# niveathika/siddhi

Measured on AMD Instinct MI355X. Metric: events/sec ingested + matches/sec (partitioned pattern, 1–8 GPU); % HBM peak, higher is better.
Workload: dtype f64; 1 GPU; P3; events_per_gpu=100000000, keys_per_gpu=10000000, micro_batch=50000896, call_size=1024, parallelism=key-sharded x1, input=prepartitioned

## Files before the change

### siddhi_amd/csrc/engine_pattern.hip

```cpp
#include <algorithm>
#include <unordered_map>
#include <cmath>
#include <cstdio>
#include <cstdlib>

#include "engine.h"
#include "knobs.h"
#include "pattern_common.h"

namespace shd {

using namespace pat;

namespace {

template <bool FAST>
__global__ __launch_bounds__(kBlock) void k_prepare(const PrepArgs* __restrict__ ap, int64_t n_ext, int64_t stride,
                                                    uint32_t* __restrict__ k32, uint64_t* __restrict__ k64,
                                                    uint32_t* __restrict__ pv, int32_t* __restrict__ tso,
                                                    PrepAgg* __restrict__ blk) {
  const PrepArgs& a = *ap;
  const DExprSet es = a.es;
  PrepAcc acc;
  const int64_t tbase = a.x.batch.ts[0];
// ... 160 lines not shown
      int64_t q = p + 1;
      int32_t j = -1;
      uint32_t fm = 0;
      int64_t ra = -1, rb = -1;
      const uint8_t st = walk_partial<true, false, HASH ? 4 : 1>(a, es, n_ext, ld, pv_row(pvp), k, tsi, q, pq, tq,
                                                                 kq, tsi, false, j, steps, viol, fm, ra, rb);
      if (st == ST_DEFER) {
        out = PS_DEFER;
        match_row[p] = (int32_t)q;
        nd++;
      } else if (st == ST_OPEN) {
        out = PS_OPEN;
        no++;
        if (a.logical == 2) match_row[p] = and_open_code(a, pv_row(pvp));
      } else if (st == ST_PRUNED) {
        pruned++;
      }
    }
    pst[p] = out;
  };
  const GlobalPos<K64, TS64> ld{skey32, skey64, spv, sts32, sts64, tbase, a.partitioned};
  for (int64_t p = t0 + threadIdx.x; p < t1; p += kBlock) visit(p, ld);
  scan_block_reduce(steps, pruned, viol, nm, no, blk, blockIdx.x, bcnt, blockIdx.x, gridDim.x, false, nd);
}

__global__ __launch_bounds__(kBlock) void k_gather_bpos(const ExtRows* __restrict__ xp, const uint32_t* spv,
                                                       int64_t n_ext) {
  const ExtRows& x = *xp;
  for (int64_t p = (int64_t)blockIdx.x * kBlock + threadIdx.x; p < n_ext; p += (int64_t)gridDim.x * kBlock) {
    const int64_t r = pv_row(spv[p]);
    const uint32_t m = r < x.C ? x.apos_mask : (x.bpos_mask | x.apos_mask);
    for (int c = 0; c < x.batch.ncols; c++) {
      if (!((m >> c) & 1u)) continue;
      const Val v = r < x.C ? col_load(x.carry, r, c) : col_load(x.batch, r - x.C, c);
      switch (x.bpos.type[c]) {
        case SHD_T_STRING: case SHD_T_INT: case SHD_T_FLOAT: ((uint32_t*)x.bpos.col[c])[p] = (uint32_t)v.b; break;
        case SHD_T_LONG: case SHD_T_DOUBLE: ((uint64_t*)x.bpos.col[c])[p] = v.b; break;
        case SHD_T_BOOL: ((uint8_t*)x.bpos.col[c])[p] = (uint8_t)v.b; break;
      }
      ((uint8_t*)x.bpos.nul[c])[p] = (uint8_t)v.null;
    }
  }
}

__global__ __launch_bounds__(kBlock) void k_block_sum(const ScanArgs* __restrict__ ap, int64_t n_ext,
                                                     const uint32_t* __restrict__ skey32,
// ... 410 lines not shown
  } else if constexpr (MODE == 1) {
    for (int64_t p = t0 + threadIdx.x; p < t1; p += kBlock)
      if (pst[p] == PS_DEFER) resume_one(p);
  } else {
    for (int64_t c0 = t0; c0 < t1; c0 += kBlock * 16) {
      const int64_t pb = c0 + (int64_t)threadIdx.x * 16;
      if (pb >= t1) continue;
      const uint4 raw = *reinterpret_cast<const uint4*>(pst + pb);
      const uint32_t wv[4] = {raw.x, raw.y, raw.z, raw.w};
      uint32_t hit = 0;
#pragma unroll
      for (int i = 0; i < 16; i++)
        if (((wv[i >> 2] >> ((i & 3) * 8)) & 255u) == PS_DEFER && pb + i < t1) hit |= 1u << i;
      while (hit) {
        const int64_t p = pb + __ffs(hit) - 1;
        hit &= hit - 1;
        resume_one(p);
      }
    }
  }
  scan_block_reduce(steps, pruned, viol, nm, no, blk, slot0 + blockIdx.x, bcnt, blockIdx.x, gridDim.x, true);
}

template <bool K64, bool FAST, bool TS64>
__global__ __launch_bounds__(kBlock) void k_resume_list(const ScanArgs* __restrict__ ap, int64_t n_ext, int64_t tile,
                                                        int ntile, const uint32_t* __restrict__ skey32,
                                                        const uint64_t* __restrict__ skey64,
                                                        const uint32_t* __restrict__ spv,
                                                        const int32_t* __restrict__ sts32,
                                                        const int64_t* __restrict__ sts64,
                                                        int32_t* __restrict__ match_row,
                                                        int32_t* __restrict__ match_other, uint8_t* __restrict__ pst,
                                                        uint32_t* __restrict__ bcnt, ScanOut* __restrict__ blk,
                                                        int slot0, const uint32_t* __restrict__ dlist,
                                                        const uint32_t* __restrict__ dcount) {
  const ScanArgs& a = *ap;
  const DExprSet es = a.es;
  uint64_t steps = 0, pruned = 0;
  uint32_t viol = 0;
  const int64_t tbase = TS64 ? 0 : a.x.batch.ts[0];
  const GlobalPos<K64, TS64> ld{skey32, skey64, spv, sts32, sts64, tbase, a.partitioned};
  const int64_t cnt = *dcount;
  for (int64_t i = (int64_t)blockIdx.x * kBlock + threadIdx.x; i < cnt; i += (int64_t)gridDim.x * kBlock) {
    const int64_t p = dlist[i];
    int64_t q = match_row[p];
    uint32_t pvp, pq;
    int64_t tsi, tq;
    uint64_t k = 0, kq = 0;
    ld(p, pvp, tsi, k);
    ld(q, pq, tq, kq);
    int32_t j = -1;
    uint32_t fm = 0;
    int64_t ra = -1, rb = -1;
    if (a.logical == 2) and_carried(a, pv_row(pvp), fm, ra, rb);
    const uint8_t st = walk_partial<false, FAST, 1, GlobalPos<K64, TS64>, 0, false>(
        a, es, n_ext, ld, pv_row(pvp), k, tsi, q, pq, tq, kq, tq, true, j, steps, viol, fm, ra, rb, p);
    uint8_t out = PS_NONE;
    const int t = (int)(p / tile);
    if (st == ST_MATCH) {
      out = PS_MATCH;
      match_row[p] = j;
      if (a.logical == 2) match_other[p] = (int32_t)((j >> kRowBits) ? ra : rb);
      atomicAdd(&bcnt[t], 1u);
    } else if (st == ST_OPEN) {
      out = PS_OPEN | PS_PEND;
      if (a.logical == 2) match_row[p] = and_code(fm, ra, rb);
      atomicAdd(&bcnt[ntile + t], 1u);
    } else if (st == ST_PRUNED) {
      pruned++;
    }
    pst[p] = out;
  }
  scan_block_reduce(steps, pruned, viol, 0u, 0u, blk, slot0 + blockIdx.x, bcnt, 0, ntile, true);
}

template <bool TS64>
__global__ __launch_bounds__(kBlock, 8) void k_lockstep_walk(const ScanArgs* __restrict__ ap, int64_t n_ext, int64_t tile,
                                                          const uint32_t* __restrict__ skey32,
                                                          const uint32_t* __restrict__ spv,
                                                          const int32_t* __restrict__ sts32,
                                                          const int64_t* __restrict__ sts64,
                                                          int32_t* __restrict__ match_row, uint8_t* __restrict__ pst,
                                                          uint32_t* __restrict__ bcnt, ScanOut* __restrict__ blk) {
  const ScanArgs& a = *ap;
  uint64_t steps = 0, pruned = 0;
  uint32_t viol = 0, nm = 0, no = 0;
  const int64_t t0 = (int64_t)blockIdx.x * tile;
  const int64_t t1 = t0 + tile < n_ext ? t0 + tile : n_ext;
  const int64_t tbase = TS64 ? 0 : a.x.batch.ts[0];
  const GlobalPos<false, TS64> ld{skey32, nullptr, spv, sts32, sts64, tbase, a.partitioned};
// ... 439 lines not shown
      ex[u] = inc - c;
      if (lane == 63) wsum[u][w] = inc;
    }
    __syncthreads();
#pragma unroll
    for (int u = 0; u < kOlU; u++) {
      uint32_t pre = 0, tot = 0;
#pragma unroll
      for (int k = 0; k < kW; k++) {
        pre += k < w ? wsum[u][k] : 0u;
        tot += wsum[u][k];
      }
      uint32_t o = base + pre + ex[u];
      const uint32_t p = (uint32_t)(c0 + u * kChunk + 4 * threadIdx.x);
#pragma unroll
      for (int b = 0; b < 4; b++)
        if ((hm[u] >> b) & 1u) olist[o++] = p + (uint32_t)b;
      base += tot;
    }
    __syncthreads();
  }
}

__global__ __launch_bounds__(kBlock) void k_gather_list(const GatherArgs* __restrict__ ap,
                                                        const uint32_t* __restrict__ olist, int64_t n_open,
                                                        const uint8_t* __restrict__ pst,
                                                        const uint32_t* __restrict__ spv,
                                                        const uint32_t* __restrict__ skey32,
                                                        const uint64_t* __restrict__ skey64) {
  const GatherArgs& a = *ap;
  const ExtRows& x = a.x;
  for (int64_t oi = (int64_t)blockIdx.x * kBlock + threadIdx.x; oi < n_open; oi = n_open) {
    const int64_t p = olist[oi];
    const int64_t o = oi;
    const int64_t r = pv_row(spv[p]);
    const uint64_t kk = !a.partitioned ? 0 : (a.key64 ? skey64[p] : (uint64_t)skey32[p]);
    const bool sts = a.sts32 || a.sts64;
    if (r < x.C) {
      for (int c = 0; c < a.ncols; c++) {
        if (!((a.amask >> c) & 1u)) continue;
        if (c == a.key_attr) {
          store_col(a.dcol[c], a.types[c], o, kk);
          a.dnul[c][o] = 0;
          continue;
        }
        const Val v = col_load(x.carry, r, c);
        store_col(a.dcol[c], a.types[c], o, v.b);
        a.dnul[c][o] = (uint8_t)v.null;
      }
      if (!sts) a.dts[o] = gld(x.carry.ts, r);
      a.dseq[o] = x.carry_seq[r];
    } else {
      const int64_t br = r - x.C;
      for (int c = 0; c < a.ncols; c++) {
        if (!((a.amask >> c) & 1u)) continue;
        if (c == a.key_attr) {
          store_col(a.dcol[c], a.types[c], o, kk);
          a.dnul[c][o] = 0;
          continue;
        }
        const Val v = col_load(x.batch, br, c);
        store_col(a.dcol[c], a.types[c], o, v.b);
        a.dnul[c][o] = (uint8_t)v.null;
      }
      if (!sts) a.dts[o] = gld(x.batch.ts, br);
      a.dseq[o] = x.seq0 + br;
    }
    if (sts) a.dts[o] = a.sts64 ? a.sts64[p] : gld(x.batch.ts, 0) + (int64_t)a.sts32[p];
    a.dkey[o] = kk;
    a.dpend[o] = (uint8_t)(((pst[p] & PS_PEND) || (r < x.C && a.pend_old[r])) ? 1 : 0);
  }
}

struct CarryTable {
  DevBuf col[kMaxCols], nul[kMaxCols], ts, key, seq;
  DevBuf pend;
  DevBuf half, bcol[kMaxCols], bnul[kMaxCols], bts, bseq;
  void reserve_b(int64_t n, const std::vector<int>& types) {
    n = std::max<int64_t>(n, 1);
    half.reserve(n);
    for (size_t c = 0; c < types.size(); c++) {
      bcol[c].reserve(n * type_size(types[c]));
      bnul[c].reserve(n);
    }
    bts.reserve(n * 8);
    bseq.reserve(n * 8);
  }
  ColSet colset_b(const std::vector<int>& types, int64_t n) const {
    ColSet cs{};
    cs.ncols = (int)types.size();
    for (size_t c = 0; c < types.size(); c++) {
      cs.col[c] = bcol[c].p;
      cs.nul[c] = bnul[c].as<uint8_t>();
// ... 105 lines not shown
  uint32_t bpos_mask = 0;
  uint32_t apos_mask = 0;
  DevBuf d_bpos[kMaxCols], d_bpos_nul[kMaxCols];
  DevBuf d_bsum;
  int s_first = 1, s_second = -1;
  int64_t W = INT64_MAX;
  bool partitioned = false;
  bool implicit_key = false;
  int key_expr[2] = {-1, -1}, key_col[2] = {-1, -1}, key_type[2] = {0, 0};
  std::vector<int> outs;
  std::vector<int> typesA;
  CarryTable carry[2];
  int cur = 0;
  int64_t C = 0;
  bool have_horizon = false;
  int64_t horizon = INT64_MIN;
  int64_t t_last = INT64_MIN;
  int64_t last_b_seq = -1;
  static constexpr int64_t kPruneMinRows = 1 << 16;
  DevBuf d_kps;
  hipEvent_t ev_pg = nullptr, ev_pt = nullptr;
  const int32_t* fin_sts32 = nullptr;
  const int64_t* fin_sts64 = nullptr;
  DevBuf d_k32, d_k32_alt, d_k64, d_k64_alt, d_pv, d_pv_alt, d_ts, d_ts_alt, d_ts64, d_match, d_pst, d_bcnt, d_boff, d_pj,
      d_pi, d_pj_alt, d_pi_alt, d_sort, d_scan, d_blk, d_mother, d_se1, d_sot, d_olist, d_dlist;
  uint32_t carry_mask = ~0u;
  ReadbackBlock<PatternTotals, PatternTotalsHost> agg;

  int kind() const override { return ENG_PATTERN; }

  void reset() override {
    C = 0;
    last_b_seq = -1;
    seq = 0;
    now = INT64_MIN;
    chunk_seq = 0;
    out.count = 0;
    counters = shd_counters{};
    have_horizon = false;
    horizon = INT64_MIN;
    t_last = INT64_MIN;
  }

  void export_replay(std::vector<Replay>& parts) override {
    SHD_HIP(hipStreamSynchronize(stream));
    const CarryTable& t = carry[cur];
// ... 155 lines not shown
    const double per_w = std::min((double)n_ext, (double)n_ext * ((double)W + 1.0) / span);
    double best = exact_passes;
    int best_b = 0;
    for (int p = 1; p < exact_passes; p++) {
      const double e = per_w / std::ldexp(1.0, 8 * p);
      const double cost = p + 0.7 * e;
      if (cost < best) {
        best = cost;
        best_b = 8 * p;
      }
    }
    return best_b;
  }

  ~PatternEngine() override {
    if (ev_pg) (void)hipEventDestroy(ev_pg);
    if (ev_pt) (void)hipEventDestroy(ev_pt);
  }

  void push(const Staged& b) override {
    if (b.n <= 0) return;
    fin_sts32 = nullptr;
    fin_sts64 = nullptr;
    sort_push(b);
  }

  void sort_push(const Staged& b) {
    const int64_t n = b.n;
    if (n <= 0) return;
    const bool isA = b.stream == sA, isB = b.stream == sB;
    const int64_t n_ext = C + n;
    if (n_ext + (logical == 2 ? C : 0) > (int64_t)kRowMask)
      throw Error(SHD_E_CAPACITY, "pattern batch + carried partials exceed 2^28 rows");
    hipStream_t s = stream;
    SHD_HIP(hipEventRecord(ev0, s));
    stage_begin();
    const int slot = isA ? 0 : 1;
    const bool keyed = partitioned || implicit_key;
    const bool key64 = keyed && type_key64(key_type[slot]);
    d_pv.reserve(n_ext * 4);
    d_ts.reserve(n_ext * 4);
    if (keyed) {
      if (key64) d_k64.reserve(n_ext * 8);
      d_k32.reserve(n_ext * 4);
    }
    d_match.reserve(n_ext * 4);
// ... 67 lines not shown
                         d_k32.as<uint32_t>(), d_k64.as<uint64_t>(), d_pv.as<uint32_t>(), d_ts.as<int32_t>(),
                         d_blk.as<PrepAgg>());
    if (!fused) {
      SHD_CHECK_LAUNCH();
      hipLaunchKernelGGL(k_finish_prep, dim3(1), dim3(kBlock), 0, s, (const PrepAgg*)d_blk.as<PrepAgg>(), nblk, d_pa);
      SHD_CHECK_LAUNCH();
      agg.fetch(&PatternTotals::prep, s);
      SHD_HIP(hipStreamSynchronize(s));
    }
    PrepAgg pg = h_agg.prep;
    mark("prepare");
    if (have_horizon && (int64_t)pg.ts_min < horizon)
      throw NeedNfa("pattern engine: an event precedes the retirement horizon of an earlier push");

    const uint32_t* skey32 = nullptr;
    const uint64_t* skey64 = nullptr;
    const uint32_t* spv = d_pv.as<uint32_t>();
    const int32_t* sts32 = d_ts.as<int32_t>();
    const int64_t* sts64 = nullptr;
    bool sorted64 = false;
    const bool prune = n_ext >= kPruneMinRows && W != INT64_MAX && !partitioned;
    const bool grouped = partitioned || (implicit_key && !pg.unmono && (C == 0 || pg.carry_tmax <= pg.ts_min));
    uint32_t hash_mask = 0;
    counters.group_bits = 0;
    if (grouped) {
      const uint64_t kmin = pg.kmin <= pg.kmax ? pg.kmin : 0;
      uint64_t kmax = pg.kmax;
      int bits = 0;
      while (bits < 64 && (kmax >> bits)) bits++;
      uint32_t kbase = 0;
      if (bits <= 32 && !type_key64(key_type[slot])) {
        int rb = 0;
        while (rb < 64 && ((kmax - kmin) >> rb)) rb++;
        if (rb < bits) {
          bits = rb > 0 ? rb : 1;
          kbase = (uint32_t)kmin;
        }
      }
      bool in_alt = false;
      if (bits <= 32) {
        const int hb = hashed_bucket_bits(pg, n_ext, bits, prune && !partitioned);
        if (hb > 0) {
          bits = hb;
          hash_mask = hb >= 32 ? 0xFFFFFFFFu : ((1u << hb) - 1u);
        }
      }
// ... 7 lines not shown
      if (fused && (hash_mask || bits > 32))
        throw Error(SHD_E_DEVICE, "pattern engine: fused key sort on a hashed or wide key");
      if (bits <= 32) {
        d_k32_alt.reserve(n_ext * 4);
        if (fused)
          keyed_sort_rest(s, n_ext, bits, kbase, d_k32.as<uint32_t>(), d_pv.as<uint32_t>(), d_ts.as<uint32_t>(),
                          d_k32_alt.as<uint32_t>(), d_pv_alt.as<uint32_t>(), d_ts_alt.as<uint32_t>(), d_kps, d_sort,
                          in_alt);
        else
          radix_sort_triples_u32(d_k32.as<uint32_t>(), d_pv.as<uint32_t>(), d_ts.as<uint32_t>(),
                                 d_k32_alt.as<uint32_t>(), d_pv_alt.as<uint32_t>(), d_ts_alt.as<uint32_t>(), n_ext,
                                 bits, d_sort, s, in_alt, hash_mask != 0, hash_mask ? 0u : kbase);
        skey32 = in_alt ? d_k32_alt.as<uint32_t>() : d_k32.as<uint32_t>();
      } else {
        d_k64_alt.reserve(n_ext * 8);
        radix_sort_triples_u64(d_k64.as<uint64_t>(), d_pv.as<uint32_t>(), d_ts.as<uint32_t>(),
                               d_k64_alt.as<uint64_t>(), d_pv_alt.as<uint32_t>(), d_ts_alt.as<uint32_t>(), n_ext,
                               bits, d_sort, s, in_alt);
        skey64 = in_alt ? d_k64_alt.as<uint64_t>() : d_k64.as<uint64_t>();
        sorted64 = true;
      }
      spv = in_alt ? d_pv_alt.as<uint32_t>() : d_pv.as<uint32_t>();
      sts32 = in_alt ? d_ts_alt.as<int32_t>() : d_ts.as<int32_t>();
      mark("key_sort");
      counters.group_bits = bits;
    }
    if (fused) {
      SHD_HIP(hipEventSynchronize(ev_pt));
      pg = h_agg.prep_pass0;
    }
    if (pg.ovf || knob_on(Knob::TS64)) {
      d_ts64.reserve(n_ext * 8);
      hipLaunchKernelGGL(k_sorted_ts64, dim3(grid_cover(n_ext)), dim3(kBlock), 0, s, dev_args(x), spv, n_ext,
                         d_ts64.as<int64_t>());
      SHD_CHECK_LAUNCH();
      sts64 = d_ts64.as<int64_t>();
    }

    ScanArgs sa{};
    sa.x = x;
    sa.es = dset();
    sa.f2 = dfilters(f2);
    sa.logical = logical;
    sa.s_first = s_first;
    sa.s_second = s_second;
    if (logical) sa.f3 = dfilters(f3);
    if (logical == 2) sa.carry_half = carry[cur].half.as<uint8_t>();
    sa.within = W;
    sa.partitioned = grouped;
    sa.prune = prune;
    sa.hash_mask = hash_mask;
    const int64_t t_end = (int64_t)pg.ts_max;
    sa.t_end = t_end;
    const bool fast2 = sa.f2.fp.ok != 0 && (!logical || sa.f3.fp.ok != 0);
    const int64_t tile = ceil_div(ceil_div(n_ext, nblk), kBlock) * kBlock;
    const int ntile = (int)ceil_div(n_ext, tile);
    d_bcnt.reserve((size_t)3 * ntile * 4);
    d_boff.reserve((size_t)3 * ntile * 4);
    const bool ts64 = sts64 != nullptr;
    bool dense = !grouped;
    double e_key = 0.0;
    if (grouped) {
      const double span = (double)(pg.ts_max - pg.ts_min) + 1.0;
      const double per_w = W == INT64_MAX ? (double)n_ext : std::min((double)n_ext, (double)n_ext * ((double)W + 1.0) / span);
      const double nkeys = hash_mask ? (double)hash_mask + 1.0 : (double)(pg.kmax - std::min(pg.kmin, pg.kmax)) + 1.0;
      e_key = per_w / nkeys;
      dense = e_key >= 0.25;
    }
    int rmode = dense ? (hash_mask ? 1 : (logical != 2 ? 3 : (and_indep ? 2 : 1))) : 0;
    if (int m; knob_int(Knob::RESUME_MODE, m)) {
      if (m >= 0 && m <= 3 && !(m >= 2 && (hash_mask || (logical == 2 && (m == 3 || !and_indep))))) rmode = m;
    }
    const int ls_force = knob_force(Knob::LOCKSTEP);
    const bool lockstep = grouped && !hash_mask && !sorted64 && logical == 0 && isB && fast2 && e_key < 64.0 &&
                          (ls_force >= 0 ? ls_force != 0 : rmode == 3);
    if (grouped && (rmode != 0 || lockstep) && isB && bpos_mask && !knob_on(Knob::NO_BPOS) &&
        (e_key >= 8.0 || knob_on(Knob::BPOS))) {
      uint32_t apos = apos_mask & carry_mask;
      for (int c = 0; c < kMaxCols; c++)
        if (((apos >> c) & 1u) && (c >= b.cs.ncols || c >= (int)typesA.size() || typesA[c] != b.cs.type[c]))
          apos &= ~(1u << c);
// ... 2 lines not shown
      sa.x.apos_mask = apos;
      for (int c = 0; c < b.cs.ncols; c++) {
        if (!(((bpos_mask | apos) >> c) & 1u)) continue;
        d_bpos[c].reserve(n_ext * type_size(b.cs.type[c]));
        d_bpos_nul[c].reserve(n_ext);
        sa.x.bpos.col[c] = d_bpos[c].p;
        sa.x.bpos.nul[c] = d_bpos_nul[c].as<uint8_t>();
      }
      sa.x.bpos_mask = bpos_mask;
      hipLaunchKernelGGL(k_gather_bpos, dim3(grid_for(n_ext, 1, 4096)), dim3(kBlock), 0, s, dev_args(sa.x), spv, n_ext);
      SHD_CHECK_LAUNCH();
    }
    sa.sp = F2Split{};
    if (fast2 && logical == 0 && !knob_on(Knob::NO_SPLIT)) split_f2(sa.f2.fp, s_first, sa.x, sa.sp);
    sa.bsum = nullptr;
    const bool skip_ok = grouped && !hash_mask && !sorted64 && !ts64 && isB && logical == 0 && rmode != 0 && !lockstep &&
                         sa.f2.fp.ok && !knob_on(Knob::NO_BLOCK_SKIP) && (e_key >= 64.0 || knob_on(Knob::BLOCK_SKIP));
    if (skip_ok && block_skip_term(sa.f2.fp, s_first, sa.bs_ci, sa.bs_side, sa.bs_op, sa.bs_attr)) {
      d_bsum.reserve(ceil_div(n_ext, 64) * (int64_t)sizeof(BlockSum));
      sa.bsum = d_bsum.as<BlockSum>();
    }
    const ScanArgs* d_sa = dev_args(sa);
    const bool rlist = rmode == 0 && !lockstep && !sa.bsum && !sorted64 && !knob_on(Knob::NO_RESUME_LIST);
    const int nlb = (int)std::max<int64_t>(1, std::min<int64_t>(1024, ceil_div(n_ext, (int64_t)64 * kBlock)));
    if (sa.bsum) {
      hipLaunchKernelGGL(k_block_sum, dim3(grid_for(ceil_div(n_ext, 64) * 64, 1, 4096)), dim3(kBlock), 0, s, d_sa,
                         n_ext, skey32, spv, sts32, d_bsum.as<BlockSum>());
      SHD_CHECK_LAUNCH();
    }
#define SHD_LAUNCH_SCAN(K64, TS64, H)                                                                           \
  hipLaunchKernelGGL((k_forward_scan<K64, TS64, H>), dim3(ntile), dim3(kBlock), 0, s, d_sa, n_ext, tile, skey32,    \
                     skey64, spv, sts32, sts64, d_match.as<int32_t>(), d_pst.as<uint8_t>(), d_bcnt.as<uint32_t>(), \
                     d_blk.as<ScanOut>())
#define SHD_LAUNCH_RESUME_D(K64, FAST, TS64, D, SLOT)                                                           \
  hipLaunchKernelGGL((k_forward_resume<K64, FAST, TS64, D>), dim3(ntile), dim3(kBlock), 0, s, d_sa, n_ext, tile, \
                     skey32, skey64, spv, sts32, sts64, d_match.as<int32_t>(), d_mother.as<int32_t>(),           \
                     d_pst.as<uint8_t>(), d_bcnt.as<uint32_t>(), d_blk.as<ScanOut>(), SLOT)
#define SHD_LAUNCH_RESUME(K64, FAST, TS64)                                                                      \
  do {                                                                                                          \
    if (rmode == 3) {                                                                                           \
      SHD_LAUNCH_RESUME_D(K64, FAST, TS64, 3, ntile);                                                           \
      SHD_CHECK_LAUNCH();                                                                                       \
      SHD_LAUNCH_RESUME_D(K64, FAST, TS64, 2, 2 * ntile);                                                       \
    } else if (rmode == 2) SHD_LAUNCH_RESUME_D(K64, FAST, TS64, 2, ntile);                                      \
    else if (rmode == 1) SHD_LAUNCH_RESUME_D(K64, FAST, TS64, 1, ntile);                                        \
    else SHD_LAUNCH_RESUME_D(K64, FAST, TS64, 0, ntile);                                                        \
// ... 1 lines not shown
#define SHD_LAUNCH_RESUME2(K64, FAST) \
  if (ts64) SHD_LAUNCH_RESUME(K64, FAST, true); else SHD_LAUNCH_RESUME(K64, FAST, false)
#define SHD_LAUNCH_SKIP(D, SLOT)                                                                                 \
  hipLaunchKernelGGL((k_forward_resume<false, true, false, D, true>), dim3(ntile), dim3(kBlock), 0, s, d_sa, n_ext, \
                     tile, skey32, skey64, spv, sts32, sts64, d_match.as<int32_t>(), d_mother.as<int32_t>(),      \
                     d_pst.as<uint8_t>(), d_bcnt.as<uint32_t>(), d_blk.as<ScanOut>(), SLOT)
    if (sorted64) {
      if (ts64) SHD_LAUNCH_SCAN(true, true, false); else SHD_LAUNCH_SCAN(true, false, false);
      SHD_CHECK_LAUNCH();
      if (fast2) { SHD_LAUNCH_RESUME2(true, true); }
      else { SHD_LAUNCH_RESUME2(true, false); }
    } else {
      if (lockstep) {
        if (ts64)
          hipLaunchKernelGGL(k_lockstep_walk<true>, dim3(ntile), dim3(kBlock), 0, s, d_sa, n_ext, tile, skey32, spv,
                             sts32, sts64, d_match.as<int32_t>(), d_pst.as<uint8_t>(), d_bcnt.as<uint32_t>(),
                             d_blk.as<ScanOut>());
        else
          hipLaunchKernelGGL(k_lockstep_walk<false>, dim3(ntile), dim3(kBlock), 0, s, d_sa, n_ext, tile, skey32, spv,
                             sts32, sts64, d_match.as<int32_t>(), d_pst.as<uint8_t>(), d_bcnt.as<uint32_t>(),
                             d_blk.as<ScanOut>());
      } else if (hash_mask) {
        if (ts64) SHD_LAUNCH_SCAN(false, true, true); else SHD_LAUNCH_SCAN(false, false, true);
      } else {
        if (ts64) SHD_LAUNCH_SCAN(false, true, false); else SHD_LAUNCH_SCAN(false, false, false);
      }
      SHD_CHECK_LAUNCH();
      if (lockstep) {
        if (ts64) SHD_LAUNCH_RESUME_D(false, true, true, 2, ntile);
        else SHD_LAUNCH_RESUME_D(false, true, false, 2, ntile);
      } else if (sa.bsum) {
        if (rmode == 3) {
          SHD_LAUNCH_SKIP(3, ntile);
          SHD_CHECK_LAUNCH();
          SHD_LAUNCH_SKIP(2, 2 * ntile);
        } else if (rmode == 2) SHD_LAUNCH_SKIP(2, ntile);
        else SHD_LAUNCH_SKIP(1, ntile);
      } else if (rlist) {
        uint32_t* d_ndef = &agg.dev()->n_deferred;
        scan_exclusive_u32(d_bcnt.as<uint32_t>() + 2 * ntile, d_boff.as<uint32_t>() + 2 * ntile, ntile, d_ndef, d_scan,
                           s);
        d_dlist.reserve((size_t)n_ext * 4);
        hipLaunchKernelGGL(k_open_list, dim3(ntile), dim3(kBlock), 0, s, (const uint8_t*)d_pst.as<uint8_t>(),
                           (const uint32_t*)d_boff.as<uint32_t>(), n_ext, tile, d_dlist.as<uint32_t>(),
                           (uint32_t)PS_DEFER, 2);
        SHD_CHECK_LAUNCH();
#define SHD_LAUNCH_RLIST(FAST, TS64)                                                                               \
  hipLaunchKernelGGL((k_resume_list<false, FAST, TS64>), dim3(nlb), dim3(kBlock), 0, s, d_sa, n_ext, tile, ntile,     \
                     skey32, skey64, spv, sts32, sts64, d_match.as<int32_t>(), d_mother.as<int32_t>(),              \
                     d_pst.as<uint8_t>(), d_bcnt.as<uint32_t>(), d_blk.as<ScanOut>(), ntile,                        \
                     (const uint32_t*)d_dlist.as<uint32_t>(), (const uint32_t*)d_ndef)
        if (fast2) {
          if (ts64) SHD_LAUNCH_RLIST(true, true); else SHD_LAUNCH_RLIST(true, false);
        } else {
          if (ts64) SHD_LAUNCH_RLIST(false, true); else SHD_LAUNCH_RLIST(false, false);
        }
#undef SHD_LAUNCH_RLIST
      } else if (fast2) { SHD_LAUNCH_RESUME2(false, true); }
      else { SHD_LAUNCH_RESUME2(false, false); }
    }
#undef SHD_LAUNCH_RESUME2
#undef SHD_LAUNCH_SKIP
#undef SHD_LAUNCH_RESUME_D
#undef SHD_LAUNCH_RESUME
#undef SHD_LAUNCH_SCAN
    SHD_CHECK_LAUNCH();
    hipLaunchKernelGGL(k_finish_scan, dim3(1), dim3(kBlock), 0, s, (const ScanOut*)d_blk.as<ScanOut>(),
                       rlist ? ntile + nlb : (rmode == 3 && !lockstep ? 3 : 2) * ntile,
                       d_so);
    SHD_CHECK_LAUNCH();
    mark("forward_scan");

    scan_exclusive_u32(d_bcnt.as<uint32_t>(), d_boff.as<uint32_t>(), ntile, &agg.dev()->n_match, d_scan, s);
    scan_exclusive_u32(d_bcnt.as<uint32_t>() + ntile, d_boff.as<uint32_t>() + ntile, ntile, &agg.dev()->n_open, d_scan,
                       s);
    mark("compact");
    agg.fetch(&PatternTotals::scan, &PatternTotals::tail_, s);
    SHD_HIP(hipMemcpyAsync(&h_agg.t_last, b.cs.ts + (n - 1), 8, hipMemcpyDeviceToHost, s));
    SHD_HIP(hipStreamSynchronize(s));
    const ScanOut so = h_agg.scan;
    const uint32_t m = h_agg.n_match;
    const uint32_t n_open = h_agg.n_open;
    if (so.violation)
      throw NeedNfa("pattern engine: event timestamps decrease within a key under `within`");
    if (so.pruned) {
      have_horizon = true;
      horizon = std::max(horizon, t_end);
    }
    fin_sts32 = sts32;
    fin_sts64 = sts64;
    finish(b, x, n_ext, tile, ntile, spv, skey32, skey64, sorted64, keyed, grouped, key64, m, n_open, so, t_end,
           pg.n_cand);
  }

  void finish(const Staged& b, const ExtRows& x, int64_t n_ext, int64_t tile, int ntile, const uint32_t* spv,
              const uint32_t* skey32, const uint64_t* skey64, bool sorted64, bool keyed, bool grouped, bool key64,
              uint32_t m, uint32_t n_open, const ScanOut& so, int64_t t_end, uint64_t n_cand) {
    hipStream_t s = stream;
// ... 80 lines not shown
        for (size_t c = 0; c < typesB.size(); c++) {
          ga.typesB[c] = (int32_t)typesB[c];
          ga.dcolB[c] = carry[nxt].bcol[c].p;
          ga.dnulB[c] = carry[nxt].bnul[c].as<uint8_t>();
        }
        ga.dtsB = carry[nxt].bts.as<int64_t>();
        ga.dseqB = carry[nxt].bseq.as<int64_t>();
      }
      if (keyed && !grouped) {
        ga.key64 = key64;
        skey32 = d_k32.as<uint32_t>();
        skey64 = d_k64.as<uint64_t>();
      }
      if (logical != 2) {
        ga.amask = carry_mask;
        if (grouped) {
          ga.sts32 = fin_sts32;
          ga.sts64 = fin_sts64;
          ga.key_attr = (partitioned && !sorted64 && key_col[0] >= 0 &&
                         (key_type[0] == SHD_T_STRING || key_type[0] == SHD_T_INT)) ? key_col[0] : -1;
        } else {
          ga.key_attr = -1;
        }
        d_olist.reserve((size_t)n_open * 4);
        hipLaunchKernelGGL(k_open_list, dim3(ntile), dim3(kBlock), 0, s, (const uint8_t*)d_pst.as<uint8_t>(),
                           (const uint32_t*)d_boff.as<uint32_t>(), n_ext, tile, d_olist.as<uint32_t>(),
                           (uint32_t)PS_OPEN, 1);
        SHD_CHECK_LAUNCH();
        hipLaunchKernelGGL(k_gather_list, dim3(grid_cover((int64_t)n_open)), dim3(kBlock), 0, s, dev_args(ga),
                           (const uint32_t*)d_olist.as<uint32_t>(), (int64_t)n_open,
                           (const uint8_t*)d_pst.as<uint8_t>(), spv, skey32, skey64);
      } else {
        hipLaunchKernelGGL(k_gather_carry, dim3(ntile), dim3(kBlock), 0, s, dev_args(ga),
                           (const uint8_t*)d_pst.as<uint8_t>(), (const uint32_t*)d_boff.as<uint32_t>(), spv, skey32,
                           skey64, n_ext, tile);
      }
      SHD_CHECK_LAUNCH();
      mark("carry");
    }
    SHD_HIP(hipEventRecord(ev1, s));
    stage_end();
    SHD_HIP(hipEventSynchronize(ev1));
    float ms = 0.f;
    SHD_HIP(hipEventElapsedTime(&ms, ev0, ev1));
    cur = nxt;
    C = n_open;
    if (b.stream == sB) last_b_seq = seq + n - 1;
    seq += n;
    if (b.advance_time && t_end > now) now = t_end;
    t_last = agg.host().t_last;
    counters.events += n;
    counters.matches += m;
    counters.partial_scans += (int64_t)so.steps;
    counters.carry = C;
// ... 276 lines not shown
```

### siddhi_amd/csrc/knobs.h

```cpp
#pragma once
#include <cassert>
#include <cstdlib>

namespace shd {

#define SHD_KNOBS(X)                                                                                                  \
                                                                                                     \
  X(SYNC_CHECK, "SHD_SYNC_CHECK", FLAG, PROCESS, "synchronize after every kernel launch so a fault names its launch") \
  X(NO_FAST_PRED, "SHD_NO_FAST_PRED", FLAG, PUSH, "filters run on the expression interpreter, never pre-decoded")     \
  X(FORCE_NFA, "SHD_FORCE_NFA", FLAG, LOAD, "every state plan runs on the generic NFA engine")                        \
  X(NO_LOGICAL_SCAN, "SHD_NO_LOGICAL_SCAN", FLAG, LOAD, "`every e1 -> (e2 or/and e3)` runs on the generic NFA engine") \
  X(NO_ABSENT_SCAN, "SHD_NO_ABSENT_SCAN", FLAG, LOAD, "`every e1 -> not X for t` runs on the generic NFA engine")     \
                                                                                              \
  X(NO_HASH, "SHD_NO_HASH", FLAG, PUSH, "pattern: never sort by hashed buckets")                                      \
  X(HASH_BITS, "SHD_HASH_BITS", INT, PUSH, "pattern: sort by this many hashed-bucket bits (outside 1..32: none)")     \
  X(FUSED_SORT, "SHD_FUSED_SORT", TRISTATE, PUSH, "pattern: fused prepare + first sort pass off / on at any push size") \
  X(TS64, "SHD_TS64", FLAG, PUSH, "pattern: 64-bit sorted timestamps even when 32-bit offsets fit")                   \
  X(RESUME_MODE, "SHD_RESUME_MODE", INT, PUSH, "pattern: deferred-walk mode 0..3 (ignored where the mode cannot run)") \
  X(LOCKSTEP, "SHD_LOCKSTEP", TRISTATE, PUSH, "pattern: lockstep walks off / on wherever they can run")               \
  X(NO_BPOS, "SHD_NO_BPOS", FLAG, PUSH, "pattern: never copy e2 attributes into position order (wins over SHD_BPOS)") \
  X(BPOS, "SHD_BPOS", FLAG, PUSH, "pattern: position-major e2 attributes whenever walks are dense")                   \
  X(NO_SPLIT, "SHD_NO_SPLIT", FLAG, PUSH, "pattern: f2 through eval_fpred per step, not split per comparison")        \
  X(NO_BLOCK_SKIP, "SHD_NO_BLOCK_SKIP", FLAG, PUSH, "pattern: walks never skip 64-position blocks (wins over SHD_BLOCK_SKIP)") \
  X(BLOCK_SKIP, "SHD_BLOCK_SKIP", FLAG, PUSH, "pattern: block skipping at any key density")                           \
  X(NO_RESUME_LIST, "SHD_NO_RESUME_LIST", FLAG, PUSH, "pattern: sparse deferred walks without the compacted list")    \
  X(NO_IMPLICIT_KEY, "SHD_NO_IMPLICIT_KEY", FLAG, LOAD, "pattern: a key equality in f2 does not partition the plan")  \
                                                                                                  \
  X(KS_GENERIC_F1, "SHD_KS_GENERIC_F1", FLAG, PUSH, "fused sort: f1 through eval_fpred per row, not pre-decoded")     \
                                                                                                  \
  X(NFA_DEBUG, "SHD_NFA_DEBUG", FLAG, LOAD, "NFA: print window-lane decisions (and phase clocks in the prof build)")  \
  X(NFA_CHUNK, "SHD_NFA_CHUNK", INT, PUSH, "NFA: window-lane chunk length in events (at least 1)")                    \
  X(NFA_HASH1_ZERO, "SHD_NFA_HASH1_ZERO", FLAG, PUSH, "NFA: zero the first window-lane state hash (forces the fallback)") \
  X(NFA_WINDOW, "SHD_NFA_WINDOW", TRISTATE, LOAD, "NFA: 0 turns window lanes off")                                    \
  X(NFA_LIST, "SHD_NFA_LIST", INT, LOAD, "NFA: pending-list capacity per key (> 0)")                                  \
  X(NFA_PARTIALS, "SHD_NFA_PARTIALS", INT, LOAD, "NFA: partial capacity per key (> 0)")                               \
  X(NFA_EVENTS, "SHD_NFA_EVENTS", INT, LOAD, "NFA: event capacity per key (> 0)")                                     \
  X(NFA_RECORDS, "SHD_NFA_RECORDS", INT, LOAD, "NFA: record capacity per key (> 0)")                                  \
  X(NFA_TIMERS, "SHD_NFA_TIMERS", INT, LOAD, "NFA: timer capacity per key (> 0)")                                     \
                                                                                               \
  X(DEBUG_ARGS, "SHD_DEBUG_ARGS", FLAG, PUSH, "filter: print k_filter's arguments and stop before the launch")        \
  X(WCHUNK, "SHD_WCHUNK", FLAG, PUSH, "windows: the chunked walk (opt-in)")                                           \
  X(NO_WCHUNK, "SHD_NO_WCHUNK", FLAG, PUSH, "windows: never the chunked walk (wins over SHD_WCHUNK)")                 \
  X(NO_CALLWIN, "SHD_NO_CALLWIN", FLAG, PUSH, "windows: never the call-window path")                                  \
  X(FOLD_LANE, "SHD_FOLD_LANE", FLAG, PUSH, "group fold: one lane per group at any segment length")                   \
  X(FOLD_GENERIC, "SHD_FOLD_GENERIC", FLAG, PUSH, "group fold: the generic fold, not the sum + count one")            \
  X(EXACT_AGGREGATES, "SHD_EXACT_AGGREGATES", FLAG, LOAD, "aggregates: the in-order running fold, not segmented scans") \
  X(GROUP_DICT, "SHD_GROUP_DICT", FLAG, LOAD, "group by: the group dictionary for every key, dense ids for none")

// ... 49 lines not shown
```

Measured before the change: 23.77 billion events/s.

## Emit open and deferred record lists directly from the forward scan

```diff
diff --git a/siddhi_amd/csrc/engine_pattern.hip b/siddhi_amd/csrc/engine_pattern.hip
--- a/siddhi_amd/csrc/engine_pattern.hip
+++ b/siddhi_amd/csrc/engine_pattern.hip
@@ -206,6 +206,114 @@
   const GlobalPos<K64, TS64> ld{skey32, skey64, spv, sts32, sts64, tbase, a.partitioned};
   for (int64_t p = t0 + threadIdx.x; p < t1; p += kBlock) visit(p, ld);
   scan_block_reduce(steps, pruned, viol, nm, no, blk, blockIdx.x, bcnt, blockIdx.x, gridDim.x, false, nd);
+}
+
+constexpr int kSubPerTile = kBlock / 64;
+constexpr uint32_t kRecDeferred = 0x80000000u;
+
+constexpr int kRecRing = 128;
+__device__ __forceinline__ void wave_lds_order() {
+  __builtin_amdgcn_fence(__ATOMIC_RELEASE, "wavefront");
+  __builtin_amdgcn_wave_barrier();
+  __builtin_amdgcn_fence(__ATOMIC_ACQUIRE, "wavefront");
+}
+__global__ __launch_bounds__(kBlock) void k_forward_scan_rec(const ScanArgs* __restrict__ ap, int64_t n_ext,
+                                                             int64_t tile, const uint32_t* __restrict__ skey32,
+                                                             const uint32_t* __restrict__ spv,
+                                                             const int32_t* __restrict__ sts32,
+                                                             int32_t* __restrict__ match_row, uint8_t* __restrict__ pst,
+                                                             uint32_t* __restrict__ bcnt, ScanOut* __restrict__ blk,
+                                                             uint32_t* __restrict__ rkey, uint32_t* __restrict__ rpv,
+                                                             int32_t* __restrict__ rts, uint32_t* __restrict__ rpos,
+                                                             uint32_t* __restrict__ dlist, uint32_t* __restrict__ scnt) {
+  const ScanArgs& a = *ap;
+  const DExprSet es{};
+  uint64_t steps = 0, pruned = 0;
+  uint32_t viol = 0, no = 0, nd = 0;
+  const int lane = threadIdx.x & 63, w = threadIdx.x >> 6;
+  const int64_t sub = tile / kSubPerTile;
+  const int64_t t0 = (int64_t)blockIdx.x * tile;
+  const int64_t t1 = t0 + tile < n_ext ? t0 + tile : n_ext;
+  const int64_t s0 = t0 + (int64_t)w * sub;
+  const int64_t s1 = s0 + sub < t1 ? s0 + sub : t1;
+  const int64_t tbase = a.x.batch.ts[0];
+  const GlobalPos<false, false> ld{skey32, nullptr, spv, sts32, nullptr, tbase, a.partitioned};
+  const uint64_t below = ((uint64_t)1 << lane) - 1;
+  uint32_t wrec = 0, wdef = 0;
+  uint32_t wout = 0;
+  __shared__ uint32_t ring[kSubPerTile][4][kRecRing];
+  uint32_t (*rg)[kRecRing] = ring[w];
+  auto flush = [&](uint32_t cnt) {
+    wave_lds_order();
+    if ((uint32_t)lane < cnt) {
+      const uint32_t sl = (wout + (uint32_t)lane) & (kRecRing - 1);
+      const int64_t o = s0 + wout + lane;
+      rkey[o] = rg[0][sl];
+      rpv[o] = rg[1][sl];
+      rts[o] = (int32_t)rg[2][sl];
+      rpos[o] = rg[3][sl];
+    }
+    wave_lds_order();
+  };
+  for (int64_t c = s0; c < s1; c += 64) {
+    const int64_t p = c + lane;
+    uint8_t out = PS_NONE;
+    uint32_t pvp = 0;
+    int64_t tsi = 0;
+    uint64_t k = 0;
+    if (p < s1) {
+      uint32_t pq;
+      int64_t tq;
+      uint64_t kq = 0;
+      const int64_t q0 = p + 1 < n_ext ? p + 1 : n_ext - 1;
+      ld(p, pvp, tsi, k);
+      ld(q0, pq, tq, kq);
+      if (pv_flags(pvp) & F_CAND) {
+        int64_t q = p + 1;
+        int32_t j = -1;
+        uint32_t fm = 0;
+        int64_t ra = -1, rb = -1;
+        const uint8_t st = walk_partial<true, false, 1>(a, es, n_ext, ld, pv_row(pvp), k, tsi, q, pq, tq, kq, tsi,
+                                                        false, j, steps, viol, fm, ra, rb);
+        if (st == ST_DEFER) {
+          out = PS_DEFER;
+          match_row[p] = (int32_t)q;
+          nd++;
+        } else if (st == ST_OPEN) {
+          out = PS_OPEN;
+          no++;
+        } else if (st == ST_PRUNED) {
+          pruned++;
+        }
+      }
+      pst[p] = out;
+    }
+    const bool def = out == PS_DEFER, rec = def || out == PS_OPEN;
+    const uint64_t mrec = __ballot(rec), mdef = __ballot(def);
+    if (rec) {
+      const uint32_t sl = (wrec + (uint32_t)__popcll(mrec & below)) & (kRecRing - 1);
+      rg[0][sl] = (uint32_t)k;
+      rg[1][sl] = pvp;
+      rg[2][sl] = (uint32_t)(int32_t)(tsi - tbase);
+      rg[3][sl] = (uint32_t)p | (def ? kRecDeferred : 0u);
+    }
+    if (def) dlist[s0 + wdef + __popcll(mdef & below)] = (uint32_t)p;
+    wrec += (uint32_t)__popcll(mrec);
+    wdef += (uint32_t)__popcll(mdef);
+    if (wrec - wout >= 64) {
+      flush(64);
+      wout += 64;
+    }
+  }
+  if (wrec > wout) flush(wrec - wout);
+  if (lane == 0) {
+    const int64_t nsub = (int64_t)gridDim.x * kSubPerTile;
+    const int64_t st = (int64_t)blockIdx.x * kSubPerTile + w;
+    scnt[st] = wrec - wdef;
+    scnt[nsub + st] = wdef;
+    scnt[2 * nsub + st] = wrec;
+  }
+  scan_block_reduce(steps, pruned, viol, 0u, no, blk, blockIdx.x, bcnt, blockIdx.x, gridDim.x, false, nd);
 }
 
 __global__ __launch_bounds__(kBlock) void k_gather_bpos(const ExtRows* __restrict__ xp, const uint32_t* spv,
@@ -662,7 +770,7 @@
   scan_block_reduce(steps, pruned, viol, nm, no, blk, slot0 + blockIdx.x, bcnt, blockIdx.x, gridDim.x, true);
 }
 
-template <bool K64, bool FAST, bool TS64>
+template <bool K64, bool FAST, bool TS64, bool SUB = false>
 __global__ __launch_bounds__(kBlock) void k_resume_list(const ScanArgs* __restrict__ ap, int64_t n_ext, int64_t tile,
                                                         int ntile, const uint32_t* __restrict__ skey32,
                                                         const uint64_t* __restrict__ skey64,
@@ -673,7 +781,9 @@
                                                         int32_t* __restrict__ match_other, uint8_t* __restrict__ pst,
                                                         uint32_t* __restrict__ bcnt, ScanOut* __restrict__ blk,
                                                         int slot0, const uint32_t* __restrict__ dlist,
-                                                        const uint32_t* __restrict__ dcount) {
+                                                        const uint32_t* __restrict__ dcount,
+                                                        const uint32_t* __restrict__ doff, int nsub, int64_t sub,
+                                                        uint32_t* __restrict__ sopen) {
   const ScanArgs& a = *ap;
   const DExprSet es = a.es;
   uint64_t steps = 0, pruned = 0;
@@ -682,7 +792,19 @@
   const GlobalPos<K64, TS64> ld{skey32, skey64, spv, sts32, sts64, tbase, a.partitioned};
   const int64_t cnt = *dcount;
   for (int64_t i = (int64_t)blockIdx.x * kBlock + threadIdx.x; i < cnt; i += (int64_t)gridDim.x * kBlock) {
-    const int64_t p = dlist[i];
+    int sti = 0;
+    int64_t p;
+    if (SUB) {
+      int lo = 0, hi = nsub;
+      while (lo < hi) {
+        const int mid = (lo + hi) >> 1;
+        if ((int64_t)doff[mid] <= i) lo = mid + 1; else hi = mid;
+      }
+      sti = lo - 1;
+      p = dlist[(int64_t)sti * sub + (i - (int64_t)doff[sti])];
+    } else {
+      p = dlist[i];
+    }
     int64_t q = match_row[p];
     uint32_t pvp, pq;
     int64_t tsi, tq;
@@ -705,7 +827,8 @@
     } else if (st == ST_OPEN) {
       out = PS_OPEN | PS_PEND;
       if (a.logical == 2) match_row[p] = and_code(fm, ra, rb);
-      atomicAdd(&bcnt[ntile + t], 1u);
+      if (SUB) atomicAdd(&sopen[sti], 1u);
+      else atomicAdd(&bcnt[ntile + t], 1u);
     } else if (st == ST_PRUNED) {
       pruned++;
     }
@@ -1191,6 +1314,43 @@
   }
 }
 
+__device__ __forceinline__ void gather_open_row(const GatherArgs& a, int64_t o, int64_t r, uint64_t kk, bool sts,
+                                                bool pend_now) {
+  const ExtRows& x = a.x;
+  if (r < x.C) {
+    for (int c = 0; c < a.ncols; c++) {
+      if (!((a.amask >> c) & 1u)) continue;
+      if (c == a.key_attr) {
+        store_col(a.dcol[c], a.types[c], o, kk);
+        a.dnul[c][o] = 0;
+        continue;
+      }
+      const Val v = col_load(x.carry, r, c);
+      store_col(a.dcol[c], a.types[c], o, v.b);
+      a.dnul[c][o] = (uint8_t)v.null;
+    }
+    if (!sts) a.dts[o] = gld(x.carry.ts, r);
+    a.dseq[o] = x.carry_seq[r];
+  } else {
+    const int64_t br = r - x.C;
+    for (int c = 0; c < a.ncols; c++) {
+      if (!((a.amask >> c) & 1u)) continue;
+      if (c == a.key_attr) {
+        store_col(a.dcol[c], a.types[c], o, kk);
+        a.dnul[c][o] = 0;
+        continue;
+      }
+      const Val v = col_load(x.batch, br, c);
+      store_col(a.dcol[c], a.types[c], o, v.b);
+      a.dnul[c][o] = (uint8_t)v.null;
+    }
+    if (!sts) a.dts[o] = gld(x.batch.ts, br);
+    a.dseq[o] = x.seq0 + br;
+  }
+  a.dkey[o] = kk;
+  a.dpend[o] = (uint8_t)((pend_now || (r < x.C && a.pend_old[r])) ? 1 : 0);
+}
+
 __global__ __launch_bounds__(kBlock) void k_gather_list(const GatherArgs* __restrict__ ap,
                                                         const uint32_t* __restrict__ olist, int64_t n_open,
                                                         const uint8_t* __restrict__ pst,
@@ -1205,39 +1365,46 @@
     const int64_t r = pv_row(spv[p]);
     const uint64_t kk = !a.partitioned ? 0 : (a.key64 ? skey64[p] : (uint64_t)skey32[p]);
     const bool sts = a.sts32 || a.sts64;
-    if (r < x.C) {
-      for (int c = 0; c < a.ncols; c++) {
-        if (!((a.amask >> c) & 1u)) continue;
-        if (c == a.key_attr) {
-          store_col(a.dcol[c], a.types[c], o, kk);
-          a.dnul[c][o] = 0;
-          continue;
-        }
-        const Val v = col_load(x.carry, r, c);
-        store_col(a.dcol[c], a.types[c], o, v.b);
-        a.dnul[c][o] = (uint8_t)v.null;
-      }
-      if (!sts) a.dts[o] = gld(x.carry.ts, r);
-      a.dseq[o] = x.carry_seq[r];
-    } else {
-      const int64_t br = r - x.C;
-      for (int c = 0; c < a.ncols; c++) {
-        if (!((a.amask >> c) & 1u)) continue;
-        if (c == a.key_attr) {
-          store_col(a.dcol[c], a.types[c], o, kk);
-          a.dnul[c][o] = 0;
-          continue;
-        }
-        const Val v = col_load(x.batch, br, c);
-        store_col(a.dcol[c], a.types[c], o, v.b);
-        a.dnul[c][o] = (uint8_t)v.null;
-      }
-      if (!sts) a.dts[o] = gld(x.batch.ts, br);
-      a.dseq[o] = x.seq0 + br;
-    }
+    gather_open_row(a, o, r, kk, sts, (pst[p] & PS_PEND) != 0);
     if (sts) a.dts[o] = a.sts64 ? a.sts64[p] : gld(x.batch.ts, 0) + (int64_t)a.sts32[p];
-    a.dkey[o] = kk;
-    a.dpend[o] = (uint8_t)(((pst[p] & PS_PEND) || (r < x.C && a.pend_old[r])) ? 1 : 0);
+  }
+}
+
+__global__ __launch_bounds__(kBlock) void k_gather_rec(const GatherArgs* __restrict__ ap, int64_t sub, int nsub,
+                                                       const uint32_t* __restrict__ rkey,
+                                                       const uint32_t* __restrict__ rpv,
+                                                       const int32_t* __restrict__ rts,
+                                                       const uint32_t* __restrict__ rpos,
+                                                       const uint32_t* __restrict__ scnt,
+                                                       const uint32_t* __restrict__ soff,
+                                                       const uint8_t* __restrict__ pst) {
+  const GatherArgs& a = *ap;
+  const int lane = threadIdx.x & 63;
+  const int st = (int)blockIdx.x * kSubPerTile + (threadIdx.x >> 6);
+  const int64_t base = (int64_t)st * sub;
+  const uint32_t nrec = scnt[2 * (int64_t)nsub + st];
+  const int64_t tbase = gld(a.x.batch.ts, 0);
+  const uint64_t below = ((uint64_t)1 << lane) - 1;
+  int64_t o0 = soff[st];
+  for (uint32_t i0 = 0; i0 < nrec; i0 += 64) {
+    const uint32_t i = i0 + lane;
+    bool valid = false, pend = false;
+    if (i < nrec) {
+      const uint32_t rp = rpos[base + i];
+      valid = true;
+      if (rp & kRecDeferred) {
+        const uint8_t ps = pst[rp & ~kRecDeferred];
+        valid = (ps & 0x7Fu) == PS_OPEN;
+        pend = (ps & PS_PEND) != 0;
+      }
+    }
+    const uint64_t mv = __ballot(valid);
+    if (valid) {
+      const int64_t o = o0 + __popcll(mv & below);
+      gather_open_row(a, o, pv_row(rpv[base + i]), a.partitioned ? (uint64_t)rkey[base + i] : 0, true, pend);
+      a.dts[o] = tbase + (int64_t)rts[base + i];
+    }
+    o0 += __popcll(mv);
   }
 }
 
@@ -1389,6 +1556,13 @@
   hipEvent_t ev_pg = nullptr, ev_pt = nullptr;
   const int32_t* fin_sts32 = nullptr;
   const int64_t* fin_sts64 = nullptr;
+  struct ScanRecs {
+    bool on = false;
+    uint32_t *key = nullptr, *pv = nullptr, *pos = nullptr;
+    int32_t* ts = nullptr;
+    int64_t sub = 0;
+    int nsub = 0;
+  } fin_rec;
   DevBuf d_k32, d_k32_alt, d_k64, d_k64_alt, d_pv, d_pv_alt, d_ts, d_ts_alt, d_ts64, d_match, d_pst, d_bcnt, d_boff, d_pj,
       d_pi, d_pj_alt, d_pi_alt, d_sort, d_scan, d_blk, d_mother, d_se1, d_sot, d_olist, d_dlist;
   uint32_t carry_mask = ~0u;
@@ -1590,6 +1764,7 @@
     if (b.n <= 0) return;
     fin_sts32 = nullptr;
     fin_sts64 = nullptr;
+    fin_rec = ScanRecs{};
     sort_push(b);
   }
 
@@ -1703,6 +1878,7 @@
     const bool prune = n_ext >= kPruneMinRows && W != INT64_MAX && !partitioned;
     const bool grouped = partitioned || (implicit_key && !pg.unmono && (C == 0 || pg.carry_tmax <= pg.ts_min));
     uint32_t hash_mask = 0;
+    bool sorted_alt = false;
     counters.group_bits = 0;
     if (grouped) {
       const uint64_t kmin = pg.kmin <= pg.kmax ? pg.kmin : 0;
@@ -1756,6 +1932,7 @@
       }
       spv = in_alt ? d_pv_alt.as<uint32_t>() : d_pv.as<uint32_t>();
       sts32 = in_alt ? d_ts_alt.as<int32_t>() : d_ts.as<int32_t>();
+      sorted_alt = in_alt;
       mark("key_sort");
       counters.group_bits = bits;
     }
@@ -1789,8 +1966,11 @@
     const bool fast2 = sa.f2.fp.ok != 0 && (!logical || sa.f3.fp.ok != 0);
     const int64_t tile = ceil_div(ceil_div(n_ext, nblk), kBlock) * kBlock;
     const int ntile = (int)ceil_div(n_ext, tile);
-    d_bcnt.reserve((size_t)3 * ntile * 4);
-    d_boff.reserve((size_t)3 * ntile * 4);
+    const int nsub = ntile * kSubPerTile;
+    d_bcnt.reserve(((size_t)3 * ntile + (size_t)3 * nsub) * 4);
+    d_boff.reserve(((size_t)3 * ntile + (size_t)3 * nsub) * 4);
+    uint32_t* d_scnt = d_bcnt.as<uint32_t>() + 3 * ntile;
+    uint32_t* d_soff = d_boff.as<uint32_t>() + 3 * ntile;
     const bool ts64 = sts64 != nullptr;
     bool dense = !grouped;
     double e_key = 0.0;
@@ -1839,6 +2019,7 @@
     }
     const ScanArgs* d_sa = dev_args(sa);
     const bool rlist = rmode == 0 && !lockstep && !sa.bsum && !sorted64 && !knob_on(Knob::NO_RESUME_LIST);
+    const bool slists = rlist && grouped && !hash_mask && !ts64 && logical != 2 && !knob_on(Knob::NO_SCAN_LISTS);
     const int nlb = (int)std::max<int64_t>(1, std::min<int64_t>(1024, ceil_div(n_ext, (int64_t)64 * kBlock)));
     if (sa.bsum) {
       hipLaunchKernelGGL(k_block_sum, dim3(grid_for(ceil_div(n_ext, 64) * 64, 1, 4096)), dim3(kBlock), 0, s, d_sa,
@@ -1886,6 +2067,19 @@
                              d_blk.as<ScanOut>());
       } else if (hash_mask) {
         if (ts64) SHD_LAUNCH_SCAN(false, true, true); else SHD_LAUNCH_SCAN(false, false, true);
+      } else if (slists) {
+        fin_rec.on = true;
+        fin_rec.key = sorted_alt ? d_k32.as<uint32_t>() : d_k32_alt.as<uint32_t>();
+        fin_rec.pv = sorted_alt ? d_pv.as<uint32_t>() : d_pv_alt.as<uint32_t>();
+        fin_rec.ts = sorted_alt ? d_ts.as<int32_t>() : d_ts_alt.as<int32_t>();
+        d_olist.reserve((size_t)n_ext * 4);
+        d_dlist.reserve((size_t)n_ext * 4);
+        fin_rec.pos = d_olist.as<uint32_t>();
+        fin_rec.sub = tile / kSubPerTile;
+        fin_rec.nsub = nsub;
+        hipLaunchKernelGGL(k_forward_scan_rec, dim3(ntile), dim3(kBlock), 0, s, d_sa, n_ext, tile, skey32, spv, sts32,
+                           d_match.as<int32_t>(), d_pst.as<uint8_t>(), d_bcnt.as<uint32_t>(), d_blk.as<ScanOut>(),
+                           fin_rec.key, fin_rec.pv, fin_rec.ts, fin_rec.pos, d_dlist.as<uint32_t>(), d_scnt);
       } else {
         if (ts64) SHD_LAUNCH_SCAN(false, true, false); else SHD_LAUNCH_SCAN(false, false, false);
       }
@@ -1900,6 +2094,17 @@
           SHD_LAUNCH_SKIP(2, 2 * ntile);
         } else if (rmode == 2) SHD_LAUNCH_SKIP(2, ntile);
         else SHD_LAUNCH_SKIP(1, ntile);
+      } else if (slists) {
+        uint32_t* d_ndef = &agg.dev()->n_deferred;
+        scan_exclusive_u32(d_scnt + nsub, d_soff + nsub, nsub, d_ndef, d_scan, s);
+#define SHD_LAUNCH_RSUB(FAST)                                                                                      \
+  hipLaunchKernelGGL((k_resume_list<false, FAST, false, true>), dim3(nlb), dim3(kBlock), 0, s, d_sa, n_ext, tile,  \
+                     ntile, skey32, skey64, spv, sts32, sts64, d_match.as<int32_t>(), d_mother.as<int32_t>(),      \
+                     d_pst.as<uint8_t>(), d_bcnt.as<uint32_t>(), d_blk.as<ScanOut>(), ntile,                       \
+                     (const uint32_t*)d_dlist.as<uint32_t>(), (const uint32_t*)d_ndef,                             \
+                     (const uint32_t*)(d_soff + nsub), nsub, fin_rec.sub, d_scnt)
+        if (fast2) SHD_LAUNCH_RSUB(true); else SHD_LAUNCH_RSUB(false);
+#undef SHD_LAUNCH_RSUB
       } else if (rlist) {
         uint32_t* d_ndef = &agg.dev()->n_deferred;
         scan_exclusive_u32(d_bcnt.as<uint32_t>() + 2 * ntile, d_boff.as<uint32_t>() + 2 * ntile, ntile, d_ndef, d_scan,
@@ -1913,7 +2118,8 @@
   hipLaunchKernelGGL((k_resume_list<false, FAST, TS64>), dim3(nlb), dim3(kBlock), 0, s, d_sa, n_ext, tile, ntile,     \
                      skey32, skey64, spv, sts32, sts64, d_match.as<int32_t>(), d_mother.as<int32_t>(),              \
                      d_pst.as<uint8_t>(), d_bcnt.as<uint32_t>(), d_blk.as<ScanOut>(), ntile,                        \
-                     (const uint32_t*)d_dlist.as<uint32_t>(), (const uint32_t*)d_ndef)
+                     (const uint32_t*)d_dlist.as<uint32_t>(), (const uint32_t*)d_ndef, (const uint32_t*)nullptr, 0,  \
+                     (int64_t)0, (uint32_t*)nullptr)
         if (fast2) {
           if (ts64) SHD_LAUNCH_RLIST(true, true); else SHD_LAUNCH_RLIST(true, false);
         } else {
@@ -1936,8 +2142,11 @@
     mark("forward_scan");
 
     scan_exclusive_u32(d_bcnt.as<uint32_t>(), d_boff.as<uint32_t>(), ntile, &agg.dev()->n_match, d_scan, s);
-    scan_exclusive_u32(d_bcnt.as<uint32_t>() + ntile, d_boff.as<uint32_t>() + ntile, ntile, &agg.dev()->n_open, d_scan,
-                       s);
+    if (slists)
+      scan_exclusive_u32(d_scnt, d_soff, nsub, &agg.dev()->n_open, d_scan, s);
+    else
+      scan_exclusive_u32(d_bcnt.as<uint32_t>() + ntile, d_boff.as<uint32_t>() + ntile, ntile, &agg.dev()->n_open,
+                         d_scan, s);
     mark("compact");
     agg.fetch(&PatternTotals::scan, &PatternTotals::tail_, s);
     SHD_HIP(hipMemcpyAsync(&h_agg.t_last, b.cs.ts + (n - 1), 8, hipMemcpyDeviceToHost, s));
@@ -2064,14 +2273,23 @@
         } else {
           ga.key_attr = -1;
         }
-        d_olist.reserve((size_t)n_open * 4);
-        hipLaunchKernelGGL(k_open_list, dim3(ntile), dim3(kBlock), 0, s, (const uint8_t*)d_pst.as<uint8_t>(),
-                           (const uint32_t*)d_boff.as<uint32_t>(), n_ext, tile, d_olist.as<uint32_t>(),
-                           (uint32_t)PS_OPEN, 1);
-        SHD_CHECK_LAUNCH();
-        hipLaunchKernelGGL(k_gather_list, dim3(grid_cover((int64_t)n_open)), dim3(kBlock), 0, s, dev_args(ga),
-                           (const uint32_t*)d_olist.as<uint32_t>(), (int64_t)n_open,
-                           (const uint8_t*)d_pst.as<uint8_t>(), spv, skey32, skey64);
+        if (fin_rec.on) {
+          hipLaunchKernelGGL(k_gather_rec, dim3(ntile), dim3(kBlock), 0, s, dev_args(ga), fin_rec.sub, fin_rec.nsub,
+                             (const uint32_t*)fin_rec.key, (const uint32_t*)fin_rec.pv, (const int32_t*)fin_rec.ts,
+                             (const uint32_t*)fin_rec.pos,
+                             (const uint32_t*)(d_bcnt.as<uint32_t>() + 3 * ntile),
+                             (const uint32_t*)(d_boff.as<uint32_t>() + 3 * ntile),
+                             (const uint8_t*)d_pst.as<uint8_t>());
+        } else {
+          d_olist.reserve((size_t)n_open * 4);
+          hipLaunchKernelGGL(k_open_list, dim3(ntile), dim3(kBlock), 0, s, (const uint8_t*)d_pst.as<uint8_t>(),
+                             (const uint32_t*)d_boff.as<uint32_t>(), n_ext, tile, d_olist.as<uint32_t>(),
+                             (uint32_t)PS_OPEN, 1);
+          SHD_CHECK_LAUNCH();
+          hipLaunchKernelGGL(k_gather_list, dim3(grid_cover((int64_t)n_open)), dim3(kBlock), 0, s, dev_args(ga),
+                             (const uint32_t*)d_olist.as<uint32_t>(), (int64_t)n_open,
+                             (const uint8_t*)d_pst.as<uint8_t>(), spv, skey32, skey64);
+        }
       } else {
         hipLaunchKernelGGL(k_gather_carry, dim3(ntile), dim3(kBlock), 0, s, dev_args(ga),
                            (const uint8_t*)d_pst.as<uint8_t>(), (const uint32_t*)d_boff.as<uint32_t>(), spv, skey32,
diff --git a/siddhi_amd/csrc/knobs.h b/siddhi_amd/csrc/knobs.h
--- a/siddhi_amd/csrc/knobs.h
+++ b/siddhi_amd/csrc/knobs.h
@@ -24,6 +24,7 @@
   X(NO_BLOCK_SKIP, "SHD_NO_BLOCK_SKIP", FLAG, PUSH, "pattern: walks never skip 64-position blocks (wins over SHD_BLOCK_SKIP)") \
   X(BLOCK_SKIP, "SHD_BLOCK_SKIP", FLAG, PUSH, "pattern: block skipping at any key density")                           \
   X(NO_RESUME_LIST, "SHD_NO_RESUME_LIST", FLAG, PUSH, "pattern: sparse deferred walks without the compacted list")    \
+  X(NO_SCAN_LISTS, "SHD_NO_SCAN_LISTS", FLAG, PUSH, "pattern: open and deferred lists by the list passes, not from the scan") \
   X(NO_IMPLICIT_KEY, "SHD_NO_IMPLICIT_KEY", FLAG, LOAD, "pattern: a key equality in f2 does not partition the plan")  \
                                                                                                   \
   X(KS_GENERIC_F1, "SHD_KS_GENERIC_F1", FLAG, PUSH, "fused sort: f1 through eval_fpred per row, not pre-decoded")     \
```

Result: faster. 24.46 billion events/s (median of 6 runs) (+2.9%).
